# fgiral000/gencast-flax-nnx

Measured on AMD Instinct MI355X. Metric: denoiser-calls/sec, higher is better.
Workload: dtype f16x3 (every product = 3 fp16 MFMAs on hi/lo-split f32 operands: 22-bit products, f32 accumulate; f32 storage); 1 GPU; nano-GenCast DPM-Solver++2S 20-step sample, 2.5deg grid (73x144), 1 ensemble member per GPU, batch 1; dead_call_skipped=True, grid_nodes=10512, mesh_nodes=2562, latent=256, layers=16, heads=4, ffw_hidden=2048, c_in=262, c_out=82, k_hop=8, parallelism=ensemble-dp1, broadcast=none, rccl_ranks=0, precision=f16x3, library_built_from_this_tree=True, launcher=single

## Files before the change

### gencast-flax-nnx_amd/csrc/gc_dev_common.inc

```

typedef float f32x16 __attribute__((ext_vector_type(16)));
typedef float f32x4 __attribute__((ext_vector_type(4)));

__device__ __forceinline__ f32x4 ld4(const float* p) { return *reinterpret_cast<const f32x4*>(p); }
__device__ __forceinline__ void st4(float* p, f32x4 v) { *reinterpret_cast<f32x4*>(p) = v; }

__device__ __forceinline__ f32x16 mfma32(float a, float b, f32x16 c) {
  return __builtin_amdgcn_mfma_f32_32x32x2f32(a, b, c, 0, 0, 0);
}

typedef _Float16 f16x8 __attribute__((ext_vector_type(8)));
constexpr float kLoScale = 2048.0f;
__device__ __forceinline__ float hilo(float hi, float lo) { return __builtin_fmaf(lo, 1.0f / kLoScale, hi); }

__device__ __forceinline__ f32x16 mfma16(f32x4 a, f32x4 b, f32x16 c) {
  return __builtin_amdgcn_mfma_f32_32x32x16_f16(__builtin_bit_cast(f16x8, a), __builtin_bit_cast(f16x8, b),
                                                c, 0, 0, 0);
}

constexpr float kF16Max = 65504.0f;
__device__ __forceinline__ void split16(float x, _Float16& hi, _Float16& lo) {
#pragma clang fp contract(off)
  hi = (_Float16)x;
  lo = (_Float16)((x - (float)hi) * kLoScale);
}

__device__ __forceinline__ void store_s16(float* base, size_t row, int ld, int col, float v) {
  _Float16 hi, lo;
  split16(v, hi, lo);
  _Float16* p = reinterpret_cast<_Float16*>(base + row * ld + (col & ~31)) + (col & 31);
  p[0] = hi;
  p[32] = lo;
}

__device__ __forceinline__ void store4_s16(float* base, size_t row, int ld, int col, float a, float b,
                                           float c, float d) {
  _Float16 h[4], l[4];
  split16(a, h[0], l[0]);
  split16(b, h[1], l[1]);
  split16(c, h[2], l[2]);
  split16(d, h[3], l[3]);
  typedef _Float16 f16x4 __attribute__((ext_vector_type(4)));
  _Float16* p = reinterpret_cast<_Float16*>(base + row * ld + (col & ~31)) + (col & 31);
  *reinterpret_cast<f16x4*>(p) = f16x4{h[0], h[1], h[2], h[3]};
  *reinterpret_cast<f16x4*>(p + 32) = f16x4{l[0], l[1], l[2], l[3]};
}

__device__ __forceinline__ void stage_split16(float* lds_row, int c4, f32x4 v) {
  typedef _Float16 f16x4 __attribute__((ext_vector_type(4)));
  _Float16 hi[4], lo[4];
#pragma unroll
  for (int e = 0; e < 4; ++e) split16(v[e], hi[e], lo[e]);
  _Float16* p = reinterpret_cast<_Float16*>(lds_row) + c4 * 4;
  *reinterpret_cast<f16x4*>(p) = f16x4{hi[0], hi[1], hi[2], hi[3]};
  *reinterpret_cast<f16x4*>(p + 32) = f16x4{lo[0], lo[1], lo[2], lo[3]};
}

template <bool A16>
__device__ __forceinline__ void stage16(float* lds_row, int c4, f32x4 v) {
  if constexpr (A16) {
    typedef _Float16 f16x4 __attribute__((ext_vector_type(4)));
    _Float16* p = reinterpret_cast<_Float16*>(lds_row) + c4 * 4;
    *reinterpret_cast<f16x4*>(p) = f16x4{(_Float16)v[0], (_Float16)v[1], (_Float16)v[2], (_Float16)v[3]};
  } else {
    stage_split16(lds_row, c4, v);
  }
}

typedef _Float16 h16x4 __attribute__((ext_vector_type(4)));
__device__ __forceinline__ const _Float16* as_h16(const float* p) { return reinterpret_cast<const _Float16*>(p); }
__device__ __forceinline__ _Float16* as_h16(float* p) { return reinterpret_cast<_Float16*>(p); }
__device__ __forceinline__ f32x4 ldh4(const _Float16* p) {
  const h16x4 v = *reinterpret_cast<const h16x4*>(p);
  return f32x4{(float)v[0], (float)v[1], (float)v[2], (float)v[3]};
}
__device__ __forceinline__ void sth4(_Float16* p, f32x4 v) {
  *reinterpret_cast<h16x4*>(p) = h16x4{(_Float16)v[0], (_Float16)v[1], (_Float16)v[2], (_Float16)v[3]};
}

__device__ __forceinline__ float r16(float v) { return (float)(_Float16)v; }
__device__ __forceinline__ float r16_if(float v, int on) { return on ? (float)(_Float16)v : v; }
__device__ __forceinline__ f32x4 r16_if(f32x4 v, int on) {
  if (on) {
#pragma unroll
    for (int e = 0; e < 4; ++e) v[e] = (float)(_Float16)v[e];
  }
  return v;
}

template <typename F>
__device__ __forceinline__ void with_flag(int on, F&& f) {
  if (on) f(std::true_type{});
  else f(std::false_type{});
}
template <bool ON>
__device__ __forceinline__ float r16_c(float v) {
  if constexpr (ON) return (float)(_Float16)v;
  else return v;
}
template <bool ON>
__device__ __forceinline__ f32x4 r16_c(f32x4 v) {
  if constexpr (ON) {
#pragma unroll
    for (int e = 0; e < 4; ++e) v[e] = (float)(_Float16)v[e];
  }
  return v;
}

__device__ __forceinline__ int acc_row(int g, int hh) { return (g & 3) + 8 * (g >> 2) + 4 * hh; }

__device__ __forceinline__ float wave_sum(float v) {
#pragma unroll
  for (int o = 32; o > 0; o >>= 1) v += __shfl_xor(v, o);
  return v;
}

__device__ __forceinline__ float gelu_tanh(float x) {
  const float c = 0.7978845608028654f;
  return 0.5f * x * (1.0f + tanhf(c * (x + 0.044715f * x * x * x)));
}

__device__ __forceinline__ float swish(float x) { return x * __builtin_amdgcn_rcpf(1.0f + __expf(-x)); }

__device__ __forceinline__ float gelu_tanh_fast(float x) {
  const float c0 = -1.5957691216057308f * 1.4426950408889634f;
  const float c1 = c0 * 0.044715f;
  const float e = __builtin_amdgcn_exp2f(x * __builtin_fmaf(x * x, c1, c0));
  return x * __builtin_amdgcn_rcpf(1.0f + e);
}
```

### gencast-flax-nnx_amd/csrc/gc_kernels.hip

```cpp
#include "gc_kernels.h"

#include <algorithm>
#include <atomic>
#include <type_traits>

#include <math.h>
#include <stdlib.h>

#ifdef GC_TU_A16
#define GC_TU_NS gc_a16
#else
#define GC_TU_NS gc
#endif
namespace GC_TU_NS {
#ifdef GC_TU_A16
constexpr bool kTuA16 = true;
#else
constexpr bool kTuA16 = false;
#endif

#include "gc_dev_common.inc"


struct DynLdsOnce {
// ... 1864 lines not shown
      if (grow >= g.rows) continue;
#pragma unroll
      for (int j = 0; j < 4; ++j) {
        f32x4 v;
#pragma unroll
        for (int e = 0; e < 4; ++e) {
          float x = hilo(acc[mt][4 * j + e], acc2[mt][4 * j + e]);
          x = (fabsf(x) <= kF16Max) ? x : __builtin_nanf("");
          v[e] = r16_c<RND>(x);
        }
        const int c = col_in + 8 * j + 4 * hh;
        if (which == 0) {
          if constexpr (A16) sth4(as_h16(g.out) + (size_t)grow * g.ldo + c, v);
          else st4(g.out + (size_t)grow * g.ldo + c, v);
        } else if constexpr (A16) {
          sth4(kv + (size_t)grow * (4 * D) + (size_t)(which - 1) * (2 * D) + c, v);
        } else {
          _Float16 h4[4], l4[4];
#pragma unroll
          for (int e = 0; e < 4; ++e) split16(v[e], h4[e], l4[e]);
          _Float16* dst = kv + (size_t)grow * (4 * D) + (size_t)(which - 1) * (2 * D) + c;
          *reinterpret_cast<f16x4*>(dst) = f16x4{h4[0], h4[1], h4[2], h4[3]};
          *reinterpret_cast<f16x4*>(dst + D) = f16x4{l4[0], l4[1], l4[2], l4[3]};
        }
      }
    }
    });
#ifdef GC_STAMPS
    stamp_out();
#endif
    return;
  }
  if constexpr (A16 && EPI == 0) {
    const int cb = ntile * BN + wave * 32 + 4 * hh;
#pragma unroll
    for (int j = 0; j < 4; ++j) {
      const f32x4 bv = g.bias ? ld4(g.bias + cb + 8 * j) : f32x4{0.f, 0.f, 0.f, 0.f};
#pragma unroll
      for (int mt = 0; mt < MT; ++mt) {
        const int grow = mtile * BM + mt * 32 + r;
        f32x4 v;
#pragma unroll
        for (int e = 0; e < 4; ++e) {
          float x = hilo(acc[mt][4 * j + e], acc2[mt][4 * j + e]) + bv[e];
          if (g.act) x = gelu_tanh_fast(x);
          v[e] = x;
        }
        if (grow < g.rows) {
          if (g.out_f32) st4(g.out + (size_t)grow * g.ldo + cb + 8 * j, v);
          else sth4(as_h16(g.out) + (size_t)grow * g.ldo + cb + 8 * j, v);
        }
      }
    }
#ifdef GC_STAMPS
    stamp_out();
#endif
    return;
  }
  float bias_v = bias_reg;
  asm volatile("" : "+v"(bias_v));
  float* obase = (EPI == 1 ? g.out + (size_t)z * g.rows * g.ldo : g.out) + ntile * BN + wave * 32 + r;
  auto emit = [&](auto full_c, auto act_c, auto rnd_c) {
    constexpr bool FULL = decltype(full_c)::value, ACT = decltype(act_c)::value, RND = decltype(rnd_c)::value;
#pragma unroll
    for (int mt = 0; mt < MT; ++mt) {
      const int row0 = mtile * BM + mt * 32;
#pragma unroll
      for (int q = 0; q < 16; ++q) {
        float v = hilo(acc[mt][q], acc2[mt][q]);
        const int grow = row0 + acc_row(q, hh);
        if (EPI != 1) {
          v += bias_v;
          if (ACT) v = gelu_tanh_fast(v);
        }
        if (!F32 && CLS == KC_GEMM_QKV && EPI == 0) v = (fabsf(v) <= kF16Max) ? v : __builtin_nanf("");
        if (EPI != 1) v = r16_c<RND>(v);
        if (FULL || grow < g.rows) obase[(size_t)grow * g.ldo] = v;
      }
    }
  };
  const bool full = mtile * BM + BM <= g.rows;
  const bool act = EPI != 1 && g.act;
  if (EPI != 1 && g.round16) {
    if (act) emit(std::false_type{}, std::true_type{}, std::true_type{});
    else emit(std::false_type{}, std::false_type{}, std::true_type{});
  } else if (full && act) emit(std::true_type{}, std::true_type{}, std::false_type{});
  else if (full) emit(std::true_type{}, std::false_type{}, std::false_type{});
  else if (act) emit(std::false_type{}, std::true_type{}, std::false_type{});
  else emit(std::false_type{}, std::false_type{}, std::false_type{});
#ifdef GC_STAMPS
  stamp_out();
#endif
}

template <int CLS>
static hipError_t launch_gemm_ws_c(hipStream_t s, const GemmArgs& g_in, int mt, int splits, int epi) {
  if ((mt != 1 && mt != 2) || epi < 0 || (epi > 1 && epi != 3)) return hipErrorInvalidValue;
  if (epi == 3 && (CLS != KC_GEMM_QKV || !g_in.kv16 || g_in.kv_d % 32 || g_in.n != 3 * g_in.kv_d || splits != 1 ||
                   g_in.att_S > 0 || g_in.bias))
    return hipErrorInvalidValue;
  const int KC = mt == 1 ? 256 : 128;
  const int kc = g_in.k_slice < KC ? g_in.k_slice : KC;
  if (g_in.n % 128 || kc % 64 || g_in.k_slice % 128 || g_in.k_slice % kc || g_in.lda % 4 || g_in.ldw % 16 || splits < 1)
    return hipErrorInvalidValue;
  GemmArgs g = g_in;
  g.splits = splits;
  const int BM = 32 * mt;
  const int total = ((g.rows + BM - 1) / BM) * (g.n / 128) * splits;
  if (total <= 0) return hipSuccess;
  dim3 grid((total + 7) / 8 * 8), block(256);
#define GC_WS(MT_, EPI_, AM_) \
  hipLaunchKernelGGL((gc_gemm_ws_kernel<MT_, EPI_, CLS, AM_, 4, 3, kTuA16, (kTuA16 && AM_ == 0 && MT_ == 2)>), grid, block, 0, s, g);
  if constexpr (!kTuA16) {
    if (g.f32w) {
#define GC_WS32(MT_, EPI_, AM_) hipLaunchKernelGGL((gc_gemm_ws_kernel<MT_, EPI_, CLS, AM_, 4, 3, false, false, true>), grid, block, 0, s, g);
      if (epi == 3) return hipErrorInvalidValue;
      if (g.att_S > 0) {
        if (mt != 1 || epi != 1 || g.att_S > kMaxAttnSplits) return hipErrorInvalidValue;
        GC_WS32(1, 1, 1)
      } else if (mt == 1 && epi == 0) { GC_WS32(1, 0, 0) }
      else if (mt == 1) { GC_WS32(1, 1, 0) }
      else if (epi == 0) { GC_WS32(2, 0, 0) }
      else { GC_WS32(2, 1, 0) }
#undef GC_WS32
      return hipGetLastError();
    }
  }
  if (g.att_S > 0) {
    if (mt != 1 || epi != 1 || g.att_S > kMaxAttnSplits) return hipErrorInvalidValue;
    GC_WS(1, 1, 1)
  } else if (epi == 3) {
    if constexpr (CLS == KC_GEMM_QKV) {
      if (mt == 1) { GC_WS(1, 3, 0) } else { GC_WS(2, 3, 0) }
    }
  } else if (mt == 1 && epi == 0) { GC_WS(1, 0, 0) }
  else if (mt == 1) { GC_WS(1, 1, 0) }
  else if (epi == 0) { GC_WS(2, 0, 0) }
  else { GC_WS(2, 1, 0) }
#undef GC_WS
  return hipGetLastError();
}

#ifdef GC_STAMPS
__device__ unsigned long long* g_rowop_stamps = nullptr;
hipError_t set_gemm_rowop_stamp_buffer(unsigned long long* p) {
  return hipMemcpyToSymbol(HIP_SYMBOL(g_rowop_stamps), &p, sizeof(p));
}
#define GC_RSTAMP(i) do { __builtin_amdgcn_sched_barrier(0); rst[i] = __builtin_amdgcn_s_memtime(); __builtin_amdgcn_sched_barrier(0); } while (0)
#else
#define GC_RSTAMP(i) do { } while (0)
#endif

template <int NT, int AMODE, int CLS, int RH, bool A16 = false ,
          bool F32 = false >
__global__ __launch_bounds__(512, 1) void gc_gemm_rowop_kernel(GemmArgs g, RowFuse f) {
  extern __shared__ __attribute__((aligned(16))) float smem[];
  constexpr int MT = RH > 32 ? 2 : 1;
  constexpr int R = NT == 1 ? 8 : 4;
  const int D = g.n, LDA = D + 4;
  const int tid = threadIdx.x, nthr = blockDim.x, nwave = nthr >> 6;
  const int wave = tid >> 6, lane = tid & 63, r = lane & 31, hh = lane >> 5;
  const int mtile = blockIdx.x;
#ifdef GC_STAMPS
  unsigned long long rst[8] = {0, 0, 0, 0, 0, 0, 0, 0};
  const unsigned long long rrt0 = __builtin_amdgcn_s_memrealtime();
#endif
  GC_RSTAMP(0);
  const int steps = D / 16;
  const float* wf = g.wt + (size_t)(wave * NT) * steps * 512 + lane * 4;
  const size_t cts = (size_t)steps * 512;
  f32x4 wh[R][NT], wl[R][NT];
  ws_ring_fill<NT, R>(wh, wl, wf, cts, steps);

  auto load_x_rows = [&](int rb, f32x4 (&v)[4][2]) __attribute__((always_inline)) {
#pragma unroll
    for (int k = 0; k < 4; ++k) {
      const int rr = rb + k * nwave;
      int row = mtile * RH + rr;
      if (row >= g.rows) row = g.rows - 1;
#pragma unroll
      for (int i = 0; i < 2; ++i) {
        const int c = 4 * lane + 256 * i;
        if constexpr (A16)
          v[k][i] = (c < D && rr < RH) ? ldh4(as_h16(f.x) + (size_t)row * D + c) : f32x4{0.f, 0.f, 0.f, 0.f};
        else
          v[k][i] = (c < D && rr < RH) ? ld4(f.x + (size_t)row * D + c) : f32x4{0.f, 0.f, 0.f, 0.f};
      }
    }
  };
  constexpr bool kEarly = RH == 16;
  f32x4 xpre[4][2], bpre[2], scpre[2], ofpre[2];
  if constexpr (kEarly) {
    load_x_rows(wave, xpre);
#pragma unroll
    for (int i = 0; i < 2; ++i) {
      const int c = 4 * lane + 256 * i;
      const bool in = c < D;
      bpre[i] = (in && f.bias) ? ld4(f.bias + c) : f32x4{0.f, 0.f, 0.f, 0.f};
      scpre[i] = (in && f.B == 1) ? ld4(f.cond + c) : f32x4{0.f, 0.f, 0.f, 0.f};
      ofpre[i] = (in && f.B == 1) ? ld4(f.cond + D + c) : f32x4{0.f, 0.f, 0.f, 0.f};
    }
  }

  const int ppr = D / 4;
  constexpr int UP = (RH * NT / 8) < 4 ? (RH * NT / 8) : 4;
  if constexpr (AMODE == 0 && A16) {
    const int ppr8 = D / 8;
    for (int p = tid; p < RH * ppr8; p += nthr) {
      const int row = p / ppr8, c8 = p - row * ppr8;
      int grow = mtile * RH + row;
      if (grow >= g.rows) grow = g.rows - 1;
      st4(smem + row * LDA + (c8 >> 2) * 32 + (c8 & 3) * 4,
          ld4(reinterpret_cast<const float*>(as_h16(g.a) + (size_t)grow * g.lda + c8 * 8)));
    }
  } else if constexpr (AMODE == 0) {
    for (int p0 = tid; p0 < RH * ppr; p0 += UP * nthr)
#pragma unroll
      for (int pi = 0; pi < UP; ++pi) {
        const int p = p0 + pi * nthr;
        const int row = p / ppr, c4 = p - row * ppr;
        int grow = mtile * RH + row;
        if (grow >= g.rows) grow = g.rows - 1;
        if constexpr (F32) st4(smem + row * LDA + c4 * 4, ld4(g.a + (size_t)grow * g.lda + c4 * 4));
        else stage16<A16>(smem + row * LDA + (c4 >> 3) * 32, c4 & 7, ld4(g.a + (size_t)grow * g.lda + c4 * 4));
      }
  }
  if constexpr (AMODE == 0) {
    if (g.att_tiles) {
      constexpr int N = kItemPieces, PB = 4;
      typedef float f32x2 __attribute__((ext_vector_type(2)));
      const int row_lo = mtile * RH, row_hi = (row_lo + RH < g.rows) ? row_lo + RH : g.rows;
      for (int tt = row_lo / kTileM; tt * kTileM < row_hi; ++tt) {
        const int np = g.att_tiles[2 * tt + 1];
        if (np == 0) continue;
        const int slot_first = g.att_tiles[2 * tt];
        __syncthreads();
        const int r0 = (tt * kTileM > row_lo ? tt * kTileM : row_lo), r1 = ((tt + 1) * kTileM < row_hi ? (tt + 1) * kTileM : row_hi);
        const int npc = (r1 - r0) * ppr;
        for (int p0 = tid; p0 < npc; p0 += PB * nthr) {
          f32x4 po[PB][N];
          f32x2 ml[PB][N];
#pragma unroll
          for (int pi = 0; pi < PB; ++pi) {
            int p = p0 + pi * nthr;
            if (p >= npc) p = npc - 1;
            const int rr = p / ppr, c4 = p - rr * ppr;
            const int node = r0 + rr, col = c4 * 4;
            const int head = col / g.att_DH, dv = col - head * g.att_DH;
            const int q = node - tt * kTileM;
#pragma unroll
            for (int sp = 0; sp < N; ++sp) {
              const int spc = sp < np ? sp : np - 1;
              const size_t slot = (size_t)(slot_first + spc) * g.att_H + head;
              po[pi][sp] = ld4(g.att_po + slot * (kTileM * g.att_DH) + q * g.att_DH + dv);
              ml[pi][sp] = *reinterpret_cast<const f32x2*>(g.att_pml + slot * (kTileM * 2) + q * 2);
            }
          }
#pragma unroll
          for (int pi = 0; pi < PB; ++pi) {
            int p = p0 + pi * nthr;
            if (p >= npc) p = npc - 1;
            const int rr = p / ppr, c4 = p - rr * ppr;
            const int row = r0 + rr - row_lo;
            float mstar = -1e30f;
#pragma unroll
            for (int sp = 0; sp < N; ++sp) mstar = fmaxf(mstar, sp < np ? ml[pi][sp][0] : -1e30f);
            f32x4 acc4 = {0.f, 0.f, 0.f, 0.f};
            float lsum = 0.f;
#pragma unroll
            for (int sp = 0; sp < N; ++sp) {
              const float w = (sp < np && ml[pi][sp][1] != 0.f) ? __expf(ml[pi][sp][0] - mstar) : 0.f;
              acc4 += po[pi][sp] * w;
              lsum += w * ml[pi][sp][1];
            }
            f32x4 v = acc4 * ((lsum != 0.f) ? 1.0f / lsum : 0.f);
            if (f.round16) v = r16_c<true>(v);
            if constexpr (F32) st4(smem + row * LDA + c4 * 4, v);
            else stage16<A16>(smem + row * LDA + (c4 >> 3) * 32, c4 & 7, v);
          }
        }
      }
    }
  }
  if constexpr (AMODE != 0) {
    auto merge_pass = [&](auto nmax) __attribute__((always_inline)) {
      constexpr int N = decltype(nmax)::value;
      constexpr int PB = (N * UP <= 8) ? UP : (N <= 4 ? 2 : 1);
      typedef float f32x2 __attribute__((ext_vector_type(2)));
      for (int p0 = tid; p0 < RH * ppr; p0 += PB * nthr) {
        f32x4 po[PB][N];
        f32x2 ml[PB][N];
#pragma unroll
        for (int pi = 0; pi < PB; ++pi) {
          const int p = p0 + pi * nthr;
          const int row = p / ppr, c4 = p - row * ppr;
          int grow = mtile * RH + row;
          if (grow >= g.rows) grow = g.rows - 1;
          const int col = c4 * 4;
          const int node = grow / g.att_B, bb = grow - node * g.att_B;
          const int head = col / g.att_DH, dv = col - head * g.att_DH;
          const int q = node % kTileM;
          const size_t slot0 = ((size_t)(node / kTileM) * g.att_S * g.att_B + bb) * g.att_H + head;
#pragma unroll
          for (int sp = 0; sp < N; ++sp) {
            const int spc = sp < g.att_S ? sp : g.att_S - 1;
            const size_t slot = slot0 + (size_t)spc * g.att_B * g.att_H;
            po[pi][sp] = ld4(g.att_po + slot * (kTileM * g.att_DH) + q * g.att_DH + dv);
            ml[pi][sp] = *reinterpret_cast<const f32x2*>(g.att_pml + slot * (kTileM * 2) + q * 2);
          }
        }
#pragma unroll
        for (int pi = 0; pi < PB; ++pi) {
          const int p = p0 + pi * nthr;
          const int row = p / ppr, c4 = p - row * ppr;
          float mstar = -1e30f;
#pragma unroll
          for (int sp = 0; sp < N; ++sp) mstar = fmaxf(mstar, sp < g.att_S ? ml[pi][sp][0] : -1e30f);
          f32x4 acc4 = {0.f, 0.f, 0.f, 0.f};
          float lsum = 0.f;
#pragma unroll
          for (int sp = 0; sp < N; ++sp) {
            const float w = (sp < g.att_S && ml[pi][sp][1] != 0.f) ? __expf(ml[pi][sp][0] - mstar) : 0.f;
            acc4 += po[pi][sp] * w;
            lsum += w * ml[pi][sp][1];
          }
          f32x4 v = acc4 * ((lsum != 0.f) ? 1.0f / lsum : 0.f);
          if (f.round16) v = r16_c<true>(v);
          if constexpr (F32) st4(smem + row * LDA + c4 * 4, v);
          else stage16<A16>(smem + row * LDA + (c4 >> 3) * 32, c4 & 7, v);
        }
      }
    };
    if (g.att_S <= 2) merge_pass(std::integral_constant<int, 2>{});
    else if (g.att_S == 3) merge_pass(std::integral_constant<int, 3>{});
    else if (g.att_S == 4) merge_pass(std::integral_constant<int, 4>{});
    else merge_pass(std::integral_constant<int, kMaxAttnSplits>{});
  }
  GC_RSTAMP(1);
  __syncthreads();
  GC_RSTAMP(2);

  f32x16 acc[MT][NT], accx[MT][NT];
#pragma unroll
  for (int mt = 0; mt < MT; ++mt)
#pragma unroll
    for (int nt = 0; nt < NT; ++nt)
#pragma unroll
      for (int q = 0; q < 16; ++q) {
        acc[mt][nt][q] = 0.f;
        accx[mt][nt][q] = 0.f;
      }
  {
    int s = 0;
    const float* arow = smem + r * LDA + hh * (F32 ? 8 : 4);
#pragma unroll 1
    for (int st = 0; st < steps; st += 8) {
      ws_quad<MT, NT, R, 0, A16, F32>(acc, accx, wh, wl, arow, 32 * LDA, st, wf, cts, s, steps);
      ws_quad<MT, NT, R, 4 % R, A16, F32>(acc, accx, wh, wl, arow, 32 * LDA, st + 4, wf, cts, s, steps);
    }
  }
  GC_RSTAMP(3);
  __syncthreads();
#pragma unroll
  for (int mt = 0; mt < MT; ++mt)
#pragma unroll
    for (int nt = 0; nt < NT; ++nt) {
      const int cbase = (wave * NT + nt) * 32 + 4 * hh;
#pragma unroll
      for (int j = 0; j < 4; ++j) {
        f32x4 v;
#pragma unroll
        for (int e = 0; e < 4; ++e) v[e] = hilo(acc[mt][nt][4 * j + e], accx[mt][nt][4 * j + e]);
        st4(smem + (mt * 32 + r) * LDA + cbase + 8 * j, v);
      }
    }
  __syncthreads();
  GC_RSTAMP(4);

  with_flag(f.round16, [&](auto rc) __attribute__((always_inline)) {
  constexpr bool RND = decltype(rc)::value;
  for (int rb = wave; rb < RH; rb += 4 * nwave) {
    f32x4 v[4][2];
    float s1[4], s2[4];
    if (kEarly && rb == wave) {
#pragma unroll
      for (int k = 0; k < 4; ++k)
#pragma unroll
        for (int i = 0; i < 2; ++i) v[k][i] = xpre[k][i];
    } else {
      load_x_rows(rb, v);
    }
#pragma unroll
    for (int k = 0; k < 4; ++k) {
      const int rr = rb + k * nwave;
      const int row = mtile * RH + rr;
      s1[k] = 0.f;
      s2[k] = 0.f;
#pragma unroll
      for (int i = 0; i < 2; ++i) {
        const int c = 4 * lane + 256 * i;
        if (c < D && rr < RH) {
          f32x4 a = v[k][i];
          if constexpr (kEarly) a += bpre[i];
          else if (f.bias) a += ld4(f.bias + c);
          a += ld4(smem + rr * LDA + c);
          a = r16_c<RND>(a);
          if (row < g.rows) {
            if constexpr (A16) sth4(as_h16(f.x) + (size_t)row * D + c, a);
            else st4(f.x + (size_t)row * D + c, a);
          }
          v[k][i] = a;
          s1[k] += a[0] + a[1] + a[2] + a[3];
          s2[k] += a[0] * a[0] + a[1] * a[1] + a[2] * a[2] + a[3] * a[3];
        }
      }
    }
#pragma unroll
    for (int o = 32; o > 0; o >>= 1)
#pragma unroll
      for (int k = 0; k < 4; ++k) {
        s1[k] += __shfl_xor(s1[k], o);
        s2[k] += __shfl_xor(s2[k], o);
      }
#pragma unroll
    for (int k = 0; k < 4; ++k) {
      const int rr = rb + k * nwave;
      const int row = mtile * RH + rr;
      if (rr >= RH || row >= g.rows) continue;
      const float mean = s1[k] / (float)D;
      const float var = fmaxf(s2[k] / (float)D - mean * mean, 0.f);
      const float rstd = 1.0f / sqrtf(var + 1e-6f);
      const float* cs = f.cond + (size_t)(row % f.B) * f.cond_stride;
#pragma unroll
      for (int i = 0; i < 2; ++i) {
        const int c = 4 * lane + 256 * i;
        if (c < D) {
          f32x4 sc, of;
          if (kEarly && f.B == 1) {
            sc = scpre[i];
            of = ofpre[i];
          } else {
            sc = ld4(cs + c);
            of = ld4(cs + D + c);
          }
          if constexpr (A16) {
            sth4(as_h16(f.h) + (size_t)row * D + c, (v[k][i] - mean) * rstd * sc + of);
          } else {
            st4(f.h + (size_t)row * D + c, r16_c<RND>((v[k][i] - mean) * rstd * sc + of));
          }
        }
      }
    }
  }
  });
#ifdef GC_STAMPS
  GC_RSTAMP(5);
  asm volatile("s_waitcnt vmcnt(0)" ::: "memory");
  GC_RSTAMP(6);
  rst[7] = __builtin_amdgcn_s_memrealtime() - rrt0;
  if (g_rowop_stamps && lane == 0) {
    unsigned long long* o = g_rowop_stamps + ((size_t)blockIdx.x * nwave + wave) * 8;
    for (int i = 0; i < 8; ++i) o[i] = rst[i];
  }
#endif
}

template <int CLS>
static hipError_t launch_gemm_rowop_c(hipStream_t s, const GemmArgs& g, const RowFuse& f) {
  const int D = g.n;
  if (D % 128 || D > 512 || g.k_slice != D || g.ldw != D || !f.x || !f.h || !f.cond || f.B < 1 ||
      g.att_S > kMaxAttnSplits)
    return hipErrorInvalidValue;
  const int nt = D > 256 ? 2 : 1;
  const int nthr = (D / (32 * nt)) * 64;
  const int t32 = (g.rows + 31) / 32, t48 = (g.rows + 47) / 48;
  int rh = t32 <= 128 ? 16 : 32;
  if (t32 > 256 && (t32 + 255) / 256 > (t48 + 255) / 256 && nthr == 512 && g.att_S == 0) rh = 48;
  const size_t lds = (size_t)(rh > 32 ? 64 : 32) * (D + 4) * sizeof(float);
  const int grid = (g.rows + rh - 1) / rh;
  if (grid <= 0) return hipSuccess;
#define GC_ROWOP_R(NT_, AM_, RH_)                                                                          \
  {                                                                                                        \
    if constexpr (!kTuA16) {                                                                               \
      if (g.f32w) {                                                                                        \
        static DynLdsOnce once32;                                                                          \
        if (hipError_t e = once32.ensure((const void*)gc_gemm_rowop_kernel<NT_, AM_, CLS, RH_, false, true>, 64 * 516 * 4)) return e; \
        hipLaunchKernelGGL((gc_gemm_rowop_kernel<NT_, AM_, CLS, RH_, false, true>), dim3(grid), dim3(nthr), lds, s, g, f); \
        return hipGetLastError();                                                                          \
      }                                                                                                    \
    }                                                                                                      \
    static DynLdsOnce once;                                                                                \
    if (hipError_t e = once.ensure((const void*)gc_gemm_rowop_kernel<NT_, AM_, CLS, RH_, kTuA16>, 64 * 516 * 4)) return e; \
    hipLaunchKernelGGL((gc_gemm_rowop_kernel<NT_, AM_, CLS, RH_, kTuA16>), dim3(grid), dim3(nthr), lds, s, g, f); \
  }
#define GC_ROWOP(NT_, AM_) { if (rh == 16) GC_ROWOP_R(NT_, AM_, 16) else if (rh == 48 && AM_ == 0) GC_ROWOP_R(NT_, 0, 48) else GC_ROWOP_R(NT_, AM_, 32) }
  if (nt == 1 && g.att_S > 0) GC_ROWOP(1, 1)
  else if (nt == 1) GC_ROWOP(1, 0)
  else if (g.att_S > 0) GC_ROWOP(2, 1)
  else GC_ROWOP(2, 0)
#undef GC_ROWOP
#undef GC_ROWOP_R
  return hipGetLastError();
}

hipError_t launch_gemm_rowop(hipStream_t s, int cls, const GemmArgs& g, const RowFuse& f) {
  switch (cls) {
    case KC_GEMM_OUT: return launch_gemm_rowop_c<KC_GEMM_OUT>(s, g, f);
    default: return hipErrorInvalidValue;
  }
}

template <int ND, int MT, int NWC = 4, bool A16 = false ,
          bool F32 = false >
__global__ __launch_bounds__(64 * NWC, NWC == 8 ? 2 : ((ND <= 2 && MT == 1) ? 3 : (ND * MT <= 4 ? 2 : 1))) void gc_ffw_fused_kernel(FfwArgs g) {
  extern __shared__ __attribute__((aligned(16))) float smem[];
  constexpr int D = 128 * ND, LDA = D + 4, FS = 256, LDU = FS + 4, R = 4, BM = 32 * MT;
  constexpr int NTHR = 64 * NWC, NT1 = FS / (32 * NWC), NT2 = D / (32 * NWC);
  constexpr int AP = 32 * (D / 4) / NTHR;
  float* At = smem;
  float* Ut = smem;
  const int tid = threadIdx.x, wave = tid >> 6, lane = tid & 63, r = lane & 31, hh = lane >> 5;
  const int S = g.f / FS;
  const int z = blockIdx.x % S, mtile = blockIdx.x / S;
#ifdef GC_STAMPS
  unsigned long long stamp_v[8];
  int stamp_n = 0;
#define GC_STAMP() do { stamp_v[stamp_n++] = __builtin_amdgcn_s_memtime(); } while (0)
#else
#define GC_STAMP() do { } while (0)
#endif
  GC_STAMP();

  constexpr int steps1 = D / 16;
  const float* wf1 = g.w1f + (size_t)(z * (FS / 32) + wave * NT1) * steps1 * 512 + lane * 4;
  f32x4 wh1[R][NT1], wl1[R][NT1];
  ws_ring_fill<NT1, R>(wh1, wl1, wf1, (size_t)steps1 * 512, steps1);

  if constexpr (A16) {
    static_assert(AP % 2 == 0, "fp16 piece mapping");
    f32x4 ra[MT][AP / 2];
#pragma unroll
    for (int mb = 0; mb < MT; ++mb)
#pragma unroll
      for (int i = 0; i < AP / 2; ++i) {
        const int p = tid + NTHR * i, row = mb * 32 + p / (D / 8), c8 = p % (D / 8);
        int grow = mtile * BM + row;
        if (grow >= g.rows) grow = g.rows - 1;
        ra[mb][i] = ld4(reinterpret_cast<const float*>(as_h16(g.a) + (size_t)grow * D + c8 * 8));
      }
#pragma unroll
    for (int mb = 0; mb < MT; ++mb)
#pragma unroll
      for (int i = 0; i < AP / 2; ++i) {
        const int p = tid + NTHR * i, row = mb * 32 + p / (D / 8), c8 = p % (D / 8);
        st4(At + row * LDA + (c8 >> 2) * 32 + (c8 & 3) * 4, ra[mb][i]);
      }
  } else {
    f32x4 ra[MT][AP];
#pragma unroll
    for (int mb = 0; mb < MT; ++mb)
#pragma unroll
      for (int i = 0; i < AP; ++i) {
        const int p = tid + NTHR * i, row = mb * 32 + p / (D / 4), c4 = p % (D / 4);
        int grow = mtile * BM + row;
        if (grow >= g.rows) grow = g.rows - 1;
        ra[mb][i] = ld4(g.a + (size_t)grow * D + c4 * 4);
      }
#pragma unroll
    for (int mb = 0; mb < MT; ++mb)
#pragma unroll
      for (int i = 0; i < AP; ++i) {
        const int p = tid + NTHR * i, row = mb * 32 + p / (D / 4), c4 = p % (D / 4);
        if constexpr (F32) st4(At + row * LDA + c4 * 4, ra[mb][i]);
        else stage16<A16>(At + row * LDA + (c4 >> 3) * 32, c4 & 7, ra[mb][i]);
      }
  }
  GC_STAMP();
  __syncthreads();
  GC_STAMP();

  constexpr bool kB1Early = NWC == 8;
  f32x4 b1pre[kB1Early ? NT1 : 1][4];
  if constexpr (kB1Early) {
#pragma unroll
    for (int nt = 0; nt < NT1; ++nt)
#pragma unroll
      for (int j = 0; j < 4; ++j) b1pre[nt][j] = ld4(g.b1 + z * FS + (wave * NT1 + nt) * 32 + 4 * hh + 8 * j);
  }

  f32x16 acc1[MT][NT1], accx1[MT][NT1];
#pragma unroll
  for (int mt = 0; mt < MT; ++mt)
#pragma unroll
    for (int nt = 0; nt < NT1; ++nt)
#pragma unroll
      for (int q = 0; q < 16; ++q) {
        acc1[mt][nt][q] = 0.f;
        accx1[mt][nt][q] = 0.f;
      }
  {
    int s = 0;
    const float* arow = At + r * LDA + hh * (F32 ? 8 : 4);
#pragma unroll 1
    for (int st = 0; st < steps1; st += 4)
      ws_quad<MT, NT1, R, 0, A16, F32>(acc1, accx1, wh1, wl1, arow, 32 * LDA, st, wf1, (size_t)steps1 * 512, s, steps1);
  }
  GC_STAMP();
  const int steps2_total = g.f / 16;
  const float* wf2 = g.w2f + ((size_t)(wave * NT2) * steps2_total + (size_t)z * (FS / 16)) * 512 + lane * 4;
  const size_t cts2 = (size_t)steps2_total * 512;
  f32x4 wh2[R][NT2], wl2[R][NT2];
  ws_ring_fill<NT2, R>(wh2, wl2, wf2, cts2, FS / 16);

  typedef _Float16 f16x4 __attribute__((ext_vector_type(4)));
  typedef float f32x2v __attribute__((ext_vector_type(2)));
  f16x4 uh[NT1][4][MT], ul[NT1][4][MT];
  with_flag(g.round16, [&](auto rc) __attribute__((always_inline)) {
    constexpr bool RND = decltype(rc)::value;
#pragma unroll
    for (int nt = 0; nt < NT1; ++nt) {
      const int cbase = (wave * NT1 + nt) * 32 + 4 * hh;
#pragma unroll
      for (int j = 0; j < 4; ++j) {
        f32x4 bv;
        if constexpr (kB1Early) bv = b1pre[nt][j];
        else bv = ld4(g.b1 + z * FS + cbase + 8 * j);
#pragma unroll
        for (int mt = 0; mt < MT; ++mt) {
          _Float16 hv[4], lv[4];
          if constexpr (F32) {
            f32x4 uf;
#pragma unroll
            for (int e = 0; e < 4; ++e) uf[e] = r16_c<RND>(gelu_tanh_fast(acc1[mt][nt][4 * j + e] + bv[e]));
            uh[nt][j][mt] = __builtin_bit_cast(f16x4, f32x2v{uf[0], uf[1]});
            ul[nt][j][mt] = __builtin_bit_cast(f16x4, f32x2v{uf[2], uf[3]});
            continue;
          }
#pragma unroll
          for (int e = 0; e < 4; ++e) {
            const float u = r16_c<RND>(gelu_tanh_fast(hilo(acc1[mt][nt][4 * j + e], accx1[mt][nt][4 * j + e]) + bv[e]));
            if constexpr (A16) {
              hv[e] = (_Float16)u;
              lv[e] = (_Float16)0.f;
            } else {
              split16(u, hv[e], lv[e]);
            }
          }
          uh[nt][j][mt] = f16x4{hv[0], hv[1], hv[2], hv[3]};
          ul[nt][j][mt] = f16x4{lv[0], lv[1], lv[2], lv[3]};
        }
      }
    }
  });
  __syncthreads();
// ... 1050 lines not shown
```

Before: 763.6 calls/s.

## Add shape-specialized rowop GEMM variant with static dims, wave-mapped attention merge, DPP reductions

Adds an ST template specialization of the fused GEMM+LayerNorm row-op kernel for D=256·NT, 4 heads, batch 1. It fixes dimensions at compile time, maps attention-split merge work per wave with precomputed lane offsets instead of per-element div/mod, uses DPP-based wave reductions, and uses FMA forms for the LayerNorm statistics. The goal is to cut integer index arithmetic, shuffle cost and dynamic bounds checks in the latent-size row-op path. The risk is small rounding differences from the FMA contractions, plus extra template instantiations.

```diff
diff --git a/gencast-flax-nnx_amd/csrc/gc_dev_common.inc b/gencast-flax-nnx_amd/csrc/gc_dev_common.inc
--- a/gencast-flax-nnx_amd/csrc/gc_dev_common.inc
+++ b/gencast-flax-nnx_amd/csrc/gc_dev_common.inc
@@ -12,6 +12,26 @@
 typedef _Float16 f16x8 __attribute__((ext_vector_type(8)));
 constexpr float kLoScale = 2048.0f;
 __device__ __forceinline__ float hilo(float hi, float lo) { return __builtin_fmaf(lo, 1.0f / kLoScale, hi); }
+
+__device__ __forceinline__ float add_rounded_product(float a, float b, float c) {
+#pragma clang fp contract(off)
+  const float p = a * b;
+  return c + p;
+}
+
+template <int CTRL>
+__device__ __forceinline__ float dpp_lane(float v) {
+  return __builtin_bit_cast(float, __builtin_amdgcn_update_dpp(0, __builtin_bit_cast(int, v), CTRL, 0xf, 0xf, true));
+}
+__device__ __forceinline__ float wave_sum_xor_dpp(float v) {
+  v += __shfl_xor(v, 32);
+  v += __shfl_xor(v, 16);
+  v += dpp_lane<0x128>(v);
+  v += __shfl_xor(v, 4);
+  v += dpp_lane<0x4E>(v);
+  v += dpp_lane<0xB1>(v);
+  return v;
+}
 
 __device__ __forceinline__ f32x16 mfma16(f32x4 a, f32x4 b, f32x16 c) {
   return __builtin_amdgcn_mfma_f32_32x32x16_f16(__builtin_bit_cast(f16x8, a), __builtin_bit_cast(f16x8, b),
diff --git a/gencast-flax-nnx_amd/csrc/gc_kernels.hip b/gencast-flax-nnx_amd/csrc/gc_kernels.hip
--- a/gencast-flax-nnx_amd/csrc/gc_kernels.hip
+++ b/gencast-flax-nnx_amd/csrc/gc_kernels.hip
@@ -2040,14 +2040,32 @@
 #endif
 
 template <int NT, int AMODE, int CLS, int RH, bool A16 = false ,
-          bool F32 = false >
+          bool F32 = false ,
+          bool ST = false>
 __global__ __launch_bounds__(512, 1) void gc_gemm_rowop_kernel(GemmArgs g, RowFuse f) {
   extern __shared__ __attribute__((aligned(16))) float smem[];
   constexpr int MT = RH > 32 ? 2 : 1;
   constexpr int R = NT == 1 ? 8 : 4;
-  const int D = g.n, LDA = D + 4;
-  const int tid = threadIdx.x, nthr = blockDim.x, nwave = nthr >> 6;
-  const int wave = tid >> 6, lane = tid & 63, r = lane & 31, hh = lane >> 5;
+  constexpr int SD = 256 * NT, SH = 4, SDH = SD / SH;
+  const int D = ST ? SD : g.n, LDA = D + 4;
+  const int tid = threadIdx.x, nthr = ST ? 512 : blockDim.x, nwave = nthr >> 6;
+  const int wave = ST ? __builtin_amdgcn_readfirstlane(tid >> 6) : tid >> 6, lane = tid & 63, r = lane & 31, hh = lane >> 5;
+  [[maybe_unused]] auto lane_po = [&](int half) __attribute__((always_inline)) {
+    const unsigned col = (half * 64 + lane) * 4;
+    return (col / SDH) * (kTileM * SDH) + col % SDH;
+  };
+  auto merge_acc = [&](f32x4& acc4, float& lsum, f32x4 po, float w, float l, bool fuse_l) __attribute__((always_inline)) {
+    if constexpr (ST) {
+      acc4 = __builtin_elementwise_fma(po, f32x4{w, w, w, w}, acc4);
+      lsum = fuse_l ? __builtin_fmaf(w, l, lsum) : add_rounded_product(w, l, lsum);
+    } else {
+      acc4 += po * w;
+      lsum += w * l;
+    }
+  };
+  [[maybe_unused]] auto lane_ml = [&](int half) __attribute__((always_inline)) {
+    return ((half * 64 + lane) * 4u / SDH) * (kTileM * 2);
+  };
   const int mtile = blockIdx.x;
 #ifdef GC_STAMPS
   unsigned long long rst[8] = {0, 0, 0, 0, 0, 0, 0, 0};
@@ -2060,33 +2078,37 @@
   f32x4 wh[R][NT], wl[R][NT];
   ws_ring_fill<NT, R>(wh, wl, wf, cts, steps);
 
-  auto load_x_rows = [&](int rb, f32x4 (&v)[4][2]) __attribute__((always_inline)) {
-#pragma unroll
-    for (int k = 0; k < 4; ++k) {
+  constexpr int KR = (ST && RH == 16) ? 2 : 4, CI = (ST && NT == 1) ? 1 : 2;
+  constexpr bool kAllRows = ST && RH % (8 * KR) == 0;
+  auto load_x_rows = [&](int rb, f32x4 (&v)[KR][CI]) __attribute__((always_inline)) {
+#pragma unroll
+    for (int k = 0; k < KR; ++k) {
       const int rr = rb + k * nwave;
       int row = mtile * RH + rr;
       if (row >= g.rows) row = g.rows - 1;
 #pragma unroll
-      for (int i = 0; i < 2; ++i) {
+      for (int i = 0; i < CI; ++i) {
         const int c = 4 * lane + 256 * i;
+        const bool in = (ST || c < D) && (kAllRows || rr < RH);
         if constexpr (A16)
-          v[k][i] = (c < D && rr < RH) ? ldh4(as_h16(f.x) + (size_t)row * D + c) : f32x4{0.f, 0.f, 0.f, 0.f};
+          v[k][i] = in ? ldh4(as_h16(f.x) + (size_t)row * D + c) : f32x4{0.f, 0.f, 0.f, 0.f};
         else
-          v[k][i] = (c < D && rr < RH) ? ld4(f.x + (size_t)row * D + c) : f32x4{0.f, 0.f, 0.f, 0.f};
+          v[k][i] = in ? ld4(f.x + (size_t)row * D + c) : f32x4{0.f, 0.f, 0.f, 0.f};
       }
     }
   };
   constexpr bool kEarly = RH == 16;
-  f32x4 xpre[4][2], bpre[2], scpre[2], ofpre[2];
+  const int fB = ST ? 1 : f.B;
+  f32x4 xpre[KR][CI], bpre[CI], scpre[CI], ofpre[CI];
   if constexpr (kEarly) {
     load_x_rows(wave, xpre);
 #pragma unroll
-    for (int i = 0; i < 2; ++i) {
+    for (int i = 0; i < CI; ++i) {
       const int c = 4 * lane + 256 * i;
-      const bool in = c < D;
+      const bool in = ST || c < D;
       bpre[i] = (in && f.bias) ? ld4(f.bias + c) : f32x4{0.f, 0.f, 0.f, 0.f};
-      scpre[i] = (in && f.B == 1) ? ld4(f.cond + c) : f32x4{0.f, 0.f, 0.f, 0.f};
-      ofpre[i] = (in && f.B == 1) ? ld4(f.cond + D + c) : f32x4{0.f, 0.f, 0.f, 0.f};
+      scpre[i] = (in && fB == 1) ? ld4(f.cond + c) : f32x4{0.f, 0.f, 0.f, 0.f};
+      ofpre[i] = (in && fB == 1) ? ld4(f.cond + D + c) : f32x4{0.f, 0.f, 0.f, 0.f};
     }
   }
 
@@ -2125,31 +2147,49 @@
         __syncthreads();
         const int r0 = (tt * kTileM > row_lo ? tt * kTileM : row_lo), r1 = ((tt + 1) * kTileM < row_hi ? (tt + 1) * kTileM : row_hi);
         const int npc = (r1 - r0) * ppr;
-        for (int p0 = tid; p0 < npc; p0 += PB * nthr) {
+        for (int pb = 0; pb < npc; pb += PB * nthr) {
           f32x4 po[PB][N];
           f32x2 ml[PB][N];
+          int rrv[PB], c4v[PB];
 #pragma unroll
           for (int pi = 0; pi < PB; ++pi) {
-            int p = p0 + pi * nthr;
-            if (p >= npc) p = npc - 1;
-            const int rr = p / ppr, c4 = p - rr * ppr;
-            const int node = r0 + rr, col = c4 * 4;
-            const int head = col / g.att_DH, dv = col - head * g.att_DH;
-            const int q = node - tt * kTileM;
+            const float *pob, *mlb;
+            size_t pos, mls;
+            if constexpr (ST) {
+              int pw = (pb >> 6) + pi * 8 + wave;
+              if (pw * 64 >= npc) pw = (npc >> 6) - NT + pw % NT;
+              rrv[pi] = pw / NT;
+              c4v[pi] = (pw % NT) * 64 + lane;
+              const int q = r0 + rrv[pi] - tt * kTileM;
+              pos = (size_t)SH * kTileM * SDH;
+              mls = (size_t)SH * kTileM * 2;
+              pob = g.att_po + (size_t)slot_first * pos + q * SDH + lane_po(pw % NT);
+              mlb = g.att_pml + (size_t)slot_first * mls + q * 2 + lane_ml(pw % NT);
+            } else {
+              int p = pb + tid + pi * nthr;
+              if (p >= npc) p = npc - 1;
+              const int rr = p / ppr, c4 = p - rr * ppr;
+              rrv[pi] = rr;
+              c4v[pi] = c4;
+              const int node = r0 + rr, col = c4 * 4;
+              const int head = col / g.att_DH, dv = col - head * g.att_DH;
+              const int q = node - tt * kTileM;
+              pos = (size_t)g.att_H * (kTileM * g.att_DH);
+              mls = (size_t)g.att_H * (kTileM * 2);
+              pob = g.att_po + ((size_t)slot_first * g.att_H + head) * (kTileM * g.att_DH) + q * g.att_DH + dv;
+              mlb = g.att_pml + ((size_t)slot_first * g.att_H + head) * (kTileM * 2) + q * 2;
+            }
 #pragma unroll
             for (int sp = 0; sp < N; ++sp) {
               const int spc = sp < np ? sp : np - 1;
-              const size_t slot = (size_t)(slot_first + spc) * g.att_H + head;
-              po[pi][sp] = ld4(g.att_po + slot * (kTileM * g.att_DH) + q * g.att_DH + dv);
-              ml[pi][sp] = *reinterpret_cast<const f32x2*>(g.att_pml + slot * (kTileM * 2) + q * 2);
+              po[pi][sp] = ld4(pob + spc * pos);
+              ml[pi][sp] = *reinterpret_cast<const f32x2*>(mlb + spc * mls);
             }
           }
 #pragma unroll
           for (int pi = 0; pi < PB; ++pi) {
-            int p = p0 + pi * nthr;
-            if (p >= npc) p = npc - 1;
-            const int rr = p / ppr, c4 = p - rr * ppr;
-            const int row = r0 + rr - row_lo;
+            const int c4 = c4v[pi];
+            const int row = r0 + rrv[pi] - row_lo;
             float mstar = -1e30f;
 #pragma unroll
             for (int sp = 0; sp < N; ++sp) mstar = fmaxf(mstar, sp < np ? ml[pi][sp][0] : -1e30f);
@@ -2158,8 +2198,7 @@
 #pragma unroll
             for (int sp = 0; sp < N; ++sp) {
               const float w = (sp < np && ml[pi][sp][1] != 0.f) ? __expf(ml[pi][sp][0] - mstar) : 0.f;
-              acc4 += po[pi][sp] * w;
-              lsum += w * ml[pi][sp][1];
+              merge_acc(acc4, lsum, po[pi][sp], w, ml[pi][sp][1], true);
             }
             f32x4 v = acc4 * ((lsum != 0.f) ? 1.0f / lsum : 0.f);
             if (f.round16) v = r16_c<true>(v);
@@ -2175,32 +2214,52 @@
       constexpr int N = decltype(nmax)::value;
       constexpr int PB = (N * UP <= 8) ? UP : (N <= 4 ? 2 : 1);
       typedef float f32x2 __attribute__((ext_vector_type(2)));
-      for (int p0 = tid; p0 < RH * ppr; p0 += PB * nthr) {
+      for (int pb = 0; pb < RH * ppr; pb += PB * nthr) {
         f32x4 po[PB][N];
         f32x2 ml[PB][N];
+        int rowv[PB], c4v[PB];
 #pragma unroll
         for (int pi = 0; pi < PB; ++pi) {
-          const int p = p0 + pi * nthr;
-          const int row = p / ppr, c4 = p - row * ppr;
-          int grow = mtile * RH + row;
-          if (grow >= g.rows) grow = g.rows - 1;
-          const int col = c4 * 4;
-          const int node = grow / g.att_B, bb = grow - node * g.att_B;
-          const int head = col / g.att_DH, dv = col - head * g.att_DH;
-          const int q = node % kTileM;
-          const size_t slot0 = ((size_t)(node / kTileM) * g.att_S * g.att_B + bb) * g.att_H + head;
+          const float *pob, *mlb;
+          size_t pos, mls;
+          if constexpr (ST) {
+            const int pw = (pb >> 6) + pi * 8 + wave;
+            rowv[pi] = pw / NT;
+            c4v[pi] = (pw % NT) * 64 + lane;
+            unsigned node = mtile * RH + rowv[pi];
+            if (node >= (unsigned)g.rows) node = g.rows - 1;
+            const unsigned q = node % kTileM;
+            pos = (size_t)SH * kTileM * SDH;
+            mls = (size_t)SH * kTileM * 2;
+            pob = g.att_po + (size_t)(node / kTileM) * g.att_S * pos + q * SDH + lane_po(pw % NT);
+            mlb = g.att_pml + (size_t)(node / kTileM) * g.att_S * mls + q * 2 + lane_ml(pw % NT);
+          } else {
+            const int p = pb + tid + pi * nthr;
+            const int row = p / ppr, c4 = p - row * ppr;
+            rowv[pi] = row;
+            c4v[pi] = c4;
+            int grow = mtile * RH + row;
+            if (grow >= g.rows) grow = g.rows - 1;
+            const int col = c4 * 4;
+            const int node = grow / g.att_B, bb = grow - node * g.att_B;
+            const int head = col / g.att_DH, dv = col - head * g.att_DH;
+            const int q = node % kTileM;
+            const size_t slot0 = ((size_t)(node / kTileM) * g.att_S * g.att_B + bb) * g.att_H + head;
+            pos = (size_t)g.att_B * g.att_H * (kTileM * g.att_DH);
+            mls = (size_t)g.att_B * g.att_H * (kTileM * 2);
+            pob = g.att_po + slot0 * (kTileM * g.att_DH) + q * g.att_DH + dv;
+            mlb = g.att_pml + slot0 * (kTileM * 2) + q * 2;
+          }
 #pragma unroll
           for (int sp = 0; sp < N; ++sp) {
             const int spc = sp < g.att_S ? sp : g.att_S - 1;
-            const size_t slot = slot0 + (size_t)spc * g.att_B * g.att_H;
-            po[pi][sp] = ld4(g.att_po + slot * (kTileM * g.att_DH) + q * g.att_DH + dv);
-            ml[pi][sp] = *reinterpret_cast<const f32x2*>(g.att_pml + slot * (kTileM * 2) + q * 2);
+            po[pi][sp] = ld4(pob + spc * pos);
+            ml[pi][sp] = *reinterpret_cast<const f32x2*>(mlb + spc * mls);
           }
         }
 #pragma unroll
         for (int pi = 0; pi < PB; ++pi) {
-          const int p = p0 + pi * nthr;
-          const int row = p / ppr, c4 = p - row * ppr;
+          const int row = rowv[pi], c4 = c4v[pi];
           float mstar = -1e30f;
 #pragma unroll
           for (int sp = 0; sp < N; ++sp) mstar = fmaxf(mstar, sp < g.att_S ? ml[pi][sp][0] : -1e30f);
@@ -2209,8 +2268,7 @@
 #pragma unroll
           for (int sp = 0; sp < N; ++sp) {
             const float w = (sp < g.att_S && ml[pi][sp][1] != 0.f) ? __expf(ml[pi][sp][0] - mstar) : 0.f;
-            acc4 += po[pi][sp] * w;
-            lsum += w * ml[pi][sp][1];
+            merge_acc(acc4, lsum, po[pi][sp], w, ml[pi][sp][1], (N == 2 && sp == 1) || (N == 8 && sp >= 5));
           }
           f32x4 v = acc4 * ((lsum != 0.f) ? 1.0f / lsum : 0.f);
           if (f.round16) v = r16_c<true>(v);
@@ -2267,27 +2325,27 @@
 
   with_flag(f.round16, [&](auto rc) __attribute__((always_inline)) {
   constexpr bool RND = decltype(rc)::value;
-  for (int rb = wave; rb < RH; rb += 4 * nwave) {
-    f32x4 v[4][2];
-    float s1[4], s2[4];
+  for (int rb = wave; rb < RH; rb += KR * nwave) {
+    f32x4 v[KR][CI];
+    float s1[KR], s2[KR];
     if (kEarly && rb == wave) {
 #pragma unroll
-      for (int k = 0; k < 4; ++k)
-#pragma unroll
-        for (int i = 0; i < 2; ++i) v[k][i] = xpre[k][i];
+      for (int k = 0; k < KR; ++k)
+#pragma unroll
+        for (int i = 0; i < CI; ++i) v[k][i] = xpre[k][i];
     } else {
       load_x_rows(rb, v);
     }
 #pragma unroll
-    for (int k = 0; k < 4; ++k) {
+    for (int k = 0; k < KR; ++k) {
       const int rr = rb + k * nwave;
       const int row = mtile * RH + rr;
       s1[k] = 0.f;
       s2[k] = 0.f;
 #pragma unroll
-      for (int i = 0; i < 2; ++i) {
+      for (int i = 0; i < CI; ++i) {
         const int c = 4 * lane + 256 * i;
-        if (c < D && rr < RH) {
+        if ((ST || c < D) && (kAllRows || rr < RH)) {
           f32x4 a = v[k][i];
           if constexpr (kEarly) a += bpre[i];
           else if (f.bias) a += ld4(f.bias + c);
@@ -2299,42 +2357,64 @@
           }
           v[k][i] = a;
           s1[k] += a[0] + a[1] + a[2] + a[3];
-          s2[k] += a[0] * a[0] + a[1] * a[1] + a[2] * a[2] + a[3] * a[3];
+          if constexpr (ST)
+            s2[k] += __builtin_fmaf(a[3], a[3], __builtin_fmaf(a[2], a[2], __builtin_fmaf(a[0], a[0], a[1] * a[1])));
+          else
+            s2[k] += a[0] * a[0] + a[1] * a[1] + a[2] * a[2] + a[3] * a[3];
         }
       }
     }
-#pragma unroll
-    for (int o = 32; o > 0; o >>= 1)
-#pragma unroll
-      for (int k = 0; k < 4; ++k) {
-        s1[k] += __shfl_xor(s1[k], o);
-        s2[k] += __shfl_xor(s2[k], o);
-      }
-#pragma unroll
-    for (int k = 0; k < 4; ++k) {
+    if constexpr (ST) {
+#pragma unroll
+      for (int k = 0; k < KR; ++k) {
+        s1[k] = wave_sum_xor_dpp(s1[k]);
+        s2[k] = wave_sum_xor_dpp(s2[k]);
+      }
+    } else {
+#pragma unroll
+      for (int o = 32; o > 0; o >>= 1)
+#pragma unroll
+        for (int k = 0; k < KR; ++k) {
+          s1[k] += __shfl_xor(s1[k], o);
+          s2[k] += __shfl_xor(s2[k], o);
+        }
+    }
+#pragma unroll
+    for (int k = 0; k < KR; ++k) {
       const int rr = rb + k * nwave;
       const int row = mtile * RH + rr;
-      if (rr >= RH || row >= g.rows) continue;
-      const float mean = s1[k] / (float)D;
-      const float var = fmaxf(s2[k] / (float)D - mean * mean, 0.f);
+      if ((!kAllRows && rr >= RH) || row >= g.rows) continue;
+      float mean, var;
+      if constexpr (ST) {
+        constexpr float kInvD = 1.0f / SD;
+        static_assert((SD & (SD - 1)) == 0, "the reciprocal is exact for a power of two only");
+        mean = s1[k] * kInvD;
+        var = fmaxf(__builtin_fmaf(-mean, mean, s2[k] * kInvD), 0.f);
+      } else {
+        mean = s1[k] / (float)D;
+        var = fmaxf(s2[k] / (float)D - mean * mean, 0.f);
+      }
       const float rstd = 1.0f / sqrtf(var + 1e-6f);
-      const float* cs = f.cond + (size_t)(row % f.B) * f.cond_stride;
-#pragma unroll
-      for (int i = 0; i < 2; ++i) {
+      const float* cs = ST ? f.cond : f.cond + (size_t)(row % f.B) * f.cond_stride;
+#pragma unroll
+      for (int i = 0; i < CI; ++i) {
         const int c = 4 * lane + 256 * i;
-        if (c < D) {
+        if (ST || c < D) {
           f32x4 sc, of;
-          if (kEarly && f.B == 1) {
+          if (kEarly && fB == 1) {
             sc = scpre[i];
             of = ofpre[i];
           } else {
             sc = ld4(cs + c);
             of = ld4(cs + D + c);
           }
+          f32x4 hv;
+          if constexpr (ST) hv = __builtin_elementwise_fma((v[k][i] - mean) * rstd, sc, of);
+          else hv = (v[k][i] - mean) * rstd * sc + of;
           if constexpr (A16) {
-            sth4(as_h16(f.h) + (size_t)row * D + c, (v[k][i] - mean) * rstd * sc + of);
+            sth4(as_h16(f.h) + (size_t)row * D + c, hv);
           } else {
-            st4(f.h + (size_t)row * D + c, r16_c<RND>((v[k][i] - mean) * rstd * sc + of));
+            st4(f.h + (size_t)row * D + c, r16_c<RND>(hv));
           }
         }
       }
@@ -2367,19 +2447,26 @@
   const size_t lds = (size_t)(rh > 32 ? 64 : 32) * (D + 4) * sizeof(float);
   const int grid = (g.rows + rh - 1) / rh;
   if (grid <= 0) return hipSuccess;
-#define GC_ROWOP_R(NT_, AM_, RH_)                                                                          \
+  const bool heads4 = g.att_H == 4 && g.att_DH * 4 == D && g.att_B == 1;
+  const bool st = nthr == 512 && D == 256 * nt && f.B == 1 && (g.att_S > 0 ? heads4 : (!g.att_tiles || heads4));
+#define GC_ROWOP_K(NT_, AM_, RH_, ST_)                                                                     \
   {                                                                                                        \
     if constexpr (!kTuA16) {                                                                               \
       if (g.f32w) {                                                                                        \
         static DynLdsOnce once32;                                                                          \
-        if (hipError_t e = once32.ensure((const void*)gc_gemm_rowop_kernel<NT_, AM_, CLS, RH_, false, true>, 64 * 516 * 4)) return e; \
-        hipLaunchKernelGGL((gc_gemm_rowop_kernel<NT_, AM_, CLS, RH_, false, true>), dim3(grid), dim3(nthr), lds, s, g, f); \
+        if (hipError_t e = once32.ensure((const void*)gc_gemm_rowop_kernel<NT_, AM_, CLS, RH_, false, true, ST_>, 64 * 516 * 4)) return e; \
+        hipLaunchKernelGGL((gc_gemm_rowop_kernel<NT_, AM_, CLS, RH_, false, true, ST_>), dim3(grid), dim3(nthr), lds, s, g, f); \
         return hipGetLastError();                                                                          \
       }                                                                                                    \
     }                                                                                                      \
     static DynLdsOnce once;                                                                                \
-    if (hipError_t e = once.ensure((const void*)gc_gemm_rowop_kernel<NT_, AM_, CLS, RH_, kTuA16>, 64 * 516 * 4)) return e; \
-    hipLaunchKernelGGL((gc_gemm_rowop_kernel<NT_, AM_, CLS, RH_, kTuA16>), dim3(grid), dim3(nthr), lds, s, g, f); \
+    if (hipError_t e = once.ensure((const void*)gc_gemm_rowop_kernel<NT_, AM_, CLS, RH_, kTuA16, false, ST_>, 64 * 516 * 4)) return e; \
+    hipLaunchKernelGGL((gc_gemm_rowop_kernel<NT_, AM_, CLS, RH_, kTuA16, false, ST_>), dim3(grid), dim3(nthr), lds, s, g, f); \
+  }
+#define GC_ROWOP_R(NT_, AM_, RH_)                                                                          \
+  {                                                                                                        \
+    constexpr bool kHasSt = (NT_ == 1 && AM_ == 1 && RH_ == 16) || (NT_ == 2 && AM_ == 0 && RH_ == 48);     \
+    if (kHasSt && st) GC_ROWOP_K(NT_, AM_, RH_, kHasSt) else GC_ROWOP_K(NT_, AM_, RH_, false)              \
   }
 #define GC_ROWOP(NT_, AM_) { if (rh == 16) GC_ROWOP_R(NT_, AM_, 16) else if (rh == 48 && AM_ == 0) GC_ROWOP_R(NT_, 0, 48) else GC_ROWOP_R(NT_, AM_, 32) }
   if (nt == 1 && g.att_S > 0) GC_ROWOP(1, 1)
@@ -2388,6 +2475,7 @@
   else GC_ROWOP(2, 0)
 #undef GC_ROWOP
 #undef GC_ROWOP_R
+#undef GC_ROWOP_K
   return hipGetLastError();
 }
 
```

After: 779.3 calls/s (median of 6 runs). 1.02x the previous value.
